# chanchanchan97/ICAFusion

Hardware: NVIDIA H100
Metric: 640x512 RGB+IR pairs/sec end-to-end (higher is better)
Workload: dtype f16

## Files before the change

### icafusion_b200/csrc/conv_common.cuh

```cuda
#pragma once
#include "icaf_internal.cuh"

namespace icaf {

constexpr int BM = 128;
constexpr int BK = 64;
constexpr int kLag = 2;
constexpr int kThreads = 288;

enum AMode { A_GATHER = 0, A_TMA2D = 1, A_TMA4D = 2 };

struct ConvProblem {
  const __half* x; const float* bias; const __half* res; __half* y;
  const float* alpha; const float* beta;
  long long x_ld, res_ld, y_ld;
  const float2* ln_stats;
  const float* ln_s;
  float2* stats_out;
};
struct ConvParams {
  ConvProblem p[2];
  int M, N, K, k_pad;
  int B, Hi, Wi, Cin, Ho, Wo, kh, kw, stride, pad;
  int act, epi;
  int a_mode, tw, th, tiles_x, tiles_y;
  int stages;
  int splits;
  int cblk;
  int ln_parts;
  float ln_eps, ln_inv_k;
  int m_tiles, n_tiles, tiles;
};
struct ConvMaps {
  CUtensorMap w[2];
  CUtensorMap a[2];
  CUtensorMap y[2];
  CUtensorMap res[2];
};

__device__ __forceinline__ ConvProblem pick_problem(const ConvParams& P, unsigned z) {
  ConvProblem r;
  r.x = z ? P.p[1].x : P.p[0].x;          r.bias = z ? P.p[1].bias : P.p[0].bias;
  r.res = z ? P.p[1].res : P.p[0].res;    r.y = z ? P.p[1].y : P.p[0].y;
  r.alpha = z ? P.p[1].alpha : P.p[0].alpha; r.beta = z ? P.p[1].beta : P.p[0].beta;
  r.x_ld = z ? P.p[1].x_ld : P.p[0].x_ld; r.res_ld = z ? P.p[1].res_ld : P.p[0].res_ld;
  r.y_ld = z ? P.p[1].y_ld : P.p[0].y_ld;
  r.ln_stats = z ? P.p[1].ln_stats : P.p[0].ln_stats; r.ln_s = z ? P.p[1].ln_s : P.p[0].ln_s;
  r.stats_out = z ? P.p[1].stats_out : P.p[0].stats_out;
  return r;
}

struct TileOrigin { int m0, tb, oy0, ox0; };
__device__ __forceinline__ void tile_origin(const ConvParams& P, int mtile, int& m0, int& tb, int& oy0, int& ox0) {
  m0 = mtile * BM; tb = 0; oy0 = 0; ox0 = 0;
  if (P.a_mode == A_TMA4D) {
    const int per_img = P.tiles_x * P.tiles_y;
    m0 = 0;
    tb = mtile / per_img;
    const int t = mtile - tb * per_img;
    oy0 = (t / P.tiles_x) * P.th;
    ox0 = (t % P.tiles_x) * P.tw;
  }
}

struct EpiRow {
  float ln_a, ln_mu;
  const float* ln_s;
  float sum, sumsq;
};
__device__ __forceinline__ void epi_row_ln(EpiRow& ex, const ConvParams& P, const ConvProblem& pr, int m, bool mvalid) {
  float su = 0.f, sq = 0.f;
  if (mvalid) {
    const float2* sp = pr.ln_stats + size_t(m) * P.ln_parts;
    for (int i = 0; i < P.ln_parts; ++i) { const float2 v = __ldg(sp + i); su += v.x; sq += v.y; }
  }
  const float mu = su * P.ln_inv_k;
  ex.ln_mu = mu;
  ex.ln_a = rsqrtf(fmaxf(sq * P.ln_inv_k - mu * mu, 0.f) + P.ln_eps);
}
__device__ __forceinline__ void epi_row_emit(const EpiRow& ex, const ConvParams& P, const ConvProblem& pr, int m, int n_begin, int n_end) {
  const int slots = (P.N + 31) >> 5;
  float2* sp = pr.stats_out + size_t(m) * slots;
  const int s0 = n_begin >> 5, s1 = min((n_end + 31) >> 5, slots);
  for (int i = s0; i < s1; ++i) sp[i] = i == s0 ? make_float2(ex.sum, ex.sumsq) : make_float2(0.f, 0.f);
// ... 77 lines not shown
__device__ __forceinline__ void epi_dispatch(int mode_act, const uint32_t (&acc)[32], const float* sb, float rbias, float alpha,
                                             float beta, const __half* rp, __half* yp, bool vec, int ncols, EpiRow& ex, int cb) {
  if (XM) {
    switch (mode_act) {
      case 9: epi_chunk<0, 0, 1>(acc, sb, rbias, alpha, beta, rp, yp, vec, ncols, ex, cb); break;
      case 10: epi_chunk<2, 0, 1>(acc, sb, rbias, alpha, beta, rp, yp, vec, ncols, ex, cb); break;
      default: epi_chunk<0, 2, 2>(acc, sb, rbias, alpha, beta, rp, yp, vec, ncols, ex, cb); break;
    }
  } else {
    switch (mode_act) {
      case 0: epi_chunk<0, 0>(acc, sb, rbias, alpha, beta, rp, yp, vec, ncols, ex, cb); break;
      case 1: epi_chunk<0, 1>(acc, sb, rbias, alpha, beta, rp, yp, vec, ncols, ex, cb); break;
      case 2: epi_chunk<0, 2>(acc, sb, rbias, alpha, beta, rp, yp, vec, ncols, ex, cb); break;
      case 3: epi_chunk<1, 0>(acc, sb, rbias, alpha, beta, rp, yp, vec, ncols, ex, cb); break;
      case 4: epi_chunk<1, 1>(acc, sb, rbias, alpha, beta, rp, yp, vec, ncols, ex, cb); break;
      case 5: epi_chunk<1, 2>(acc, sb, rbias, alpha, beta, rp, yp, vec, ncols, ex, cb); break;
      case 6: epi_chunk<2, 0>(acc, sb, rbias, alpha, beta, rp, yp, vec, ncols, ex, cb); break;
      case 7: epi_chunk<2, 1>(acc, sb, rbias, alpha, beta, rp, yp, vec, ncols, ex, cb); break;
      default: epi_chunk<2, 2>(acc, sb, rbias, alpha, beta, rp, yp, vec, ncols, ex, cb); break;
    }
  }
}

struct ConvPlan {
  int kernel;
  int bn;
  unsigned grid_x, grid_y, grid_z, cluster;
  int smem;
  int tiles, m_tiles, n_tiles;
  int sms;
  bool persist;
  int ctas;
};

}
```

### icafusion_b200/csrc/conv_gemm.cu

```cuda
#include <cstdlib>
#include <cstring>

#include "conv_common.cuh"

namespace icaf {

constexpr int kMaxStages = 10;
template <int BN>
struct SmemLayout {
  static constexpr int kABytes = BM * BK * 2;
  static constexpr int kBBytes = BN * BK * 2;
  static constexpr int kStageBytes = kABytes + kBBytes;
  static constexpr int kPitch = BN + 4;
  static constexpr int kAccBytes = BM * kPitch * 4;
  static constexpr int kTailBytes = 256 + BN * 4 + 1024;
  __host__ __device__ static int region(int stages) { return stages * kStageBytes > kAccBytes ? stages * kStageBytes : kAccBytes; }
  static int total(int stages) { return region(stages) + kTailBytes; }
};


template <int BN, bool kTmaA>
__device__ __forceinline__ void load_stage(const ConvParams& P, int a_mode, uint32_t sa, uint32_t bar, uint32_t bytes,
                                           const CUtensorMap* mw, const CUtensorMap* ma, int kb, int n0, const TileOrigin& o) {
  mbar_arrive_expect_tx(bar, bytes);
  tma_load_2d(sa + SmemLayout<BN>::kABytes, mw, bar, kb * BK, n0);
  if (a_mode == A_TMA2D) {
    tma_load_2d(sa, ma, bar, kb * BK, o.m0);
  } else if (kTmaA || a_mode == A_TMA4D) {
    const int k0 = kb * BK;
    const int tap = k0 / P.Cin;
    const int ch = k0 - tap * P.Cin;
    const int ky = tap / P.kw, kx = tap - ky * P.kw;
    tma_load_4d(sa, ma, bar, ch, o.ox0 * P.stride - P.pad + kx, o.oy0 * P.stride - P.pad + ky, o.tb);
  }
}

template <int BN, bool kQuiet, class FullBar, class HandBack>
__device__ __forceinline__ int mma_loop(float (&acc0)[BN / 2], float (&acc1)[BN / 2], uint32_t smem_base, int kStages, int nkb,
                                        int s0, uint32_t ph0, FullBar full_bar, HandBack hand_back) {
  int s = s0, s_prev = s0;
  uint32_t ph = ph0;
  for (int kb = 0; kb < nkb; ++kb) {
    if (kQuiet) mbar_wait_quiet(full_bar(s), ph); else mbar_wait(full_bar(s), ph);
    const uint32_t sa = smem_base + s * SmemLayout<BN>::kStageBytes;
    wgmma_fence();
#pragma unroll
    for (int k = 0; k < BK / 16; ++k) {
      const uint64_t bd = gmma_desc_sw128(sa + SmemLayout<BN>::kABytes + 32 * k);
      wgmma_ss<0, 0>(acc0, gmma_desc_sw128(sa + 32 * k), bd, (kb | k) != 0);
      wgmma_ss<0, 0>(acc1, gmma_desc_sw128(sa + 64 * 128 + 32 * k), bd, (kb | k) != 0);
    }
    wgmma_commit();
    wgmma_wait<1>();
    if (kb > 0) hand_back(s_prev);
    s_prev = s;
    if (++s == kStages) { s = 0; ph ^= 1; }
  }
  return s_prev;
}

template <int BN, bool XM>
__global__ void __launch_bounds__(kThreads, (BN <= 64 ? 2 : 1))
conv_gemm_tc_kernel(const ConvParams P, const __grid_constant__ ConvMaps maps) {
  extern __shared__ uint8_t smem_raw[];
  const uint32_t smem_base = (smem_u32(smem_raw) + 1023u) & ~1023u;
  using L = SmemLayout<BN>;
  const int kStages = P.stages;
  const uint32_t bar_off = uint32_t(L::region(kStages));
  const uint32_t bar_base = smem_base + bar_off;
  auto full_bar = [&](int s) { return bar_base + 8u * s; };
  auto empty_bar = [&](int s) { return bar_base + 8u * (kMaxStages + s); };
  uint8_t* smem_gen = smem_raw + (smem_base - smem_u32(smem_raw));

  pdl_launch_dependents();
  const int warp = threadIdx.x >> 5;
  const int tid = threadIdx.x;
  const int splits = P.splits;
  const int mtile = splits > 1 ? blockIdx.x / splits : blockIdx.x;
  const int ntile = blockIdx.y, bz = blockIdx.z;
  const ConvProblem pr = pick_problem(P, bz);
  const int n0 = ntile * BN;
  const int a_mode = P.a_mode;
  const uint32_t crank = splits > 1 ? cluster_ctarank() : 0u;
  const int nkb_all = P.k_pad / BK;
  const int kb_begin = (nkb_all * int(crank)) / splits;
  const int nkb = (nkb_all * (int(crank) + 1)) / splits - kb_begin;
  int m0, tb, oy0, ox0;
  tile_origin(P, mtile, m0, tb, oy0, ox0);
  const TileOrigin o{m0, tb, oy0, ox0};

  if (tid == 0) {
    const uint32_t nfull = a_mode == A_GATHER ? 129u : 1u;
    for (int s = 0; s < kStages; ++s) {
      mbar_init(full_bar(s), nfull);
      mbar_init(empty_bar(s), 4);
    }
    fence_mbar_init();
  }
  if (warp == 8 && lane_id() == 0) {
    tma_prefetch_desc(bz ? &maps.w[1] : &maps.w[0]);
    if (a_mode != A_GATHER) tma_prefetch_desc(bz ? &maps.a[1] : &maps.a[0]);
  }
  float* sbias = reinterpret_cast<float*>(smem_gen + bar_off + 256);
  float* sacc = reinterpret_cast<float*>(smem_gen);
  __syncthreads();
  pdl_wait();

  if (warp < 4) {
    float bias_r[(BN + 127) / 128];
#pragma unroll
    for (int i = 0; i < (BN + 127) / 128; ++i) {
      const int col = tid + 128 * i;
      bias_r[i] = (col < BN && pr.bias && !(P.epi & ICAF_EPI_BIAS_ROW) && n0 + col < P.N) ? __ldg(pr.bias + n0 + col) : 0.f;
    }
    float alpha = 0.f, beta = 1.f;
    if (P.epi & ICAF_EPI_SCALED_RES) { alpha = __ldg(pr.alpha); beta = __ldg(pr.beta); }
    if (a_mode == A_GATHER) {
      const int lag = kStages - 2 < kLag ? kStages - 2 : kLag;
      const int c = tid & 7;
      const int r0 = tid >> 3;
      const uint32_t sw = uint32_t(c ^ (r0 & 7)) << 4;
      uint32_t base[8];
      int iy0[8], ix0[8];
#pragma unroll
      for (int i = 0; i < 8; ++i) {
        int m = o.m0 + r0 + 16 * i;
        bool mv = m < P.M;
        int mm = mv ? m : 0;
        int ox = mm % P.Wo;
        int t = mm / P.Wo;
        int oy = t % P.Ho;
        int b = t / P.Ho;
        base[i] = uint32_t(b) * uint32_t(P.Hi * P.Wi);
        iy0[i] = mv ? oy * P.stride - P.pad : -100000;
        ix0[i] = ox * P.stride - P.pad;
      }
      int s = 0, s_done = 0;
      uint32_t ph = 0;
      for (int kb = 0; kb < nkb; ++kb) {
        mbar_wait(empty_bar(s), ph ^ 1);
        const uint32_t sa = smem_base + s * L::kStageBytes;
        const int k0 = (kb_begin + kb) * BK + c * 8;
        const bool kvalid = k0 < P.K;
        const int tap = k0 / P.Cin;
        const int ch = k0 - tap * P.Cin;
        const int ky = tap / P.kw;
        const int kx = tap - ky * P.kw;
#pragma unroll
        for (int i = 0; i < 8; ++i) {
          int iy = iy0[i] + ky, ix = ix0[i] + kx;
          bool ok = kvalid && (unsigned)iy < (unsigned)P.Hi && (unsigned)ix < (unsigned)P.Wi;
          size_t off = ok ? (size_t(base[i] + uint32_t(iy * P.Wi + ix)) * size_t(pr.x_ld) + ch) : 0;
          cp_async16(sa + uint32_t(r0 + 16 * i) * 128u + sw, pr.x + off, ok);
        }
        cp_async_commit();
        if (kb >= lag) {
          if (lag == 2) cp_async_wait<2>(); else if (lag == 1) cp_async_wait<1>(); else cp_async_wait<0>();
          fence_proxy_async_smem();
          mbar_arrive(full_bar(s_done));
          if (++s_done == kStages) s_done = 0;
        }
        if (++s == kStages) { s = 0; ph ^= 1; }
      }
      cp_async_wait<0>();
      fence_proxy_async_smem();
      for (int kb = nkb - lag < 0 ? 0 : nkb - lag; kb < nkb; ++kb) {
        mbar_arrive(full_bar(s_done));
        if (++s_done == kStages) s_done = 0;
      }
    }

    const int row = tid;
    int m;
    bool mvalid;
    if (a_mode == A_TMA4D) {
      const int ry = row / P.tw, rx = row - ry * P.tw;
      m = (tb * P.Ho + oy0 + ry) * P.Wo + ox0 + rx;
      mvalid = ry < P.th && oy0 + ry < P.Ho;
    } else {
      m = m0 + row;
      mvalid = m < P.M;
    }
    const float rbias = ((P.epi & ICAF_EPI_BIAS_ROW) && pr.bias && mvalid) ? __ldg(pr.bias + m) : 0.f;
    __half* yrow = pr.y + size_t(mvalid ? m : 0) * pr.y_ld;
    const __half* rrow = pr.res ? pr.res + size_t(mvalid ? m : 0) * pr.res_ld : nullptr;
    const int mode = (P.epi & ICAF_EPI_SCALED_RES) ? 2 : (rrow ? 1 : 0);
    if (rrow && mvalid) {
      for (int cb = 0; cb < BN && n0 + cb < P.N; cb += 64) prefetch_l2(rrow + n0 + cb);
    }
#pragma unroll
    for (int i = 0; i < (BN + 127) / 128; ++i)
      if (tid + 128 * i < BN) sbias[tid + 128 * i] = bias_r[i];
    EpiRow ex;
// ... 18 lines not shown
            float4 v;
            ld_cluster_v4(peer + 16u * q, v);
            acc[4 * q] = __float_as_uint(__uint_as_float(acc[4 * q]) + v.x);
            acc[4 * q + 1] = __float_as_uint(__uint_as_float(acc[4 * q + 1]) + v.y);
            acc[4 * q + 2] = __float_as_uint(__uint_as_float(acc[4 * q + 2]) + v.z);
            acc[4 * q + 3] = __float_as_uint(__uint_as_float(acc[4 * q + 3]) + v.w);
          }
        }
        const int nb = n0 + cb;
        if (mvalid && nb < P.N) {
          const int ncols = min(32, P.N - nb);
          const bool vec = ncols == 32 && ((reinterpret_cast<uintptr_t>(yrow + nb) & 15) == 0) &&
                           (!rrow || (reinterpret_cast<uintptr_t>(rrow + nb) & 15) == 0);
          const float* sb = sbias + cb;
          const __half* rp = rrow ? rrow + nb : nullptr;
          __half* yp = yrow + nb;
          epi_dispatch<XM>(mode_act, acc, sb, rbias, alpha, beta, rp, yp, vec, ncols, ex, cb);
        }
      }
      if (XM && mode_act == 11 && mvalid && n0 < P.N) epi_row_emit(ex, P, pr, m, n0, min(n0 + BN, P.N));
    }
    if (splits > 1) { cluster_arrive(); cluster_wait(); }
  } else if (warp < 8) {
    float acc0[BN / 2], acc1[BN / 2];
#pragma unroll
    for (int i = 0; i < BN / 2; ++i) { acc0[i] = 0.f; acc1[i] = 0.f; }
    mma_loop<BN, false>(acc0, acc1, smem_base, kStages, nkb, 0, 0u, full_bar,
                        [&](int s) { if (lane_id() == 0) mbar_arrive(empty_bar(s)); });
    wgmma_wait<0>();
    const int t = tid - 128, w = t >> 5, l = t & 31;
#pragma unroll
    for (int i = 0; i < BN / 2; i += 2) {
      const int r = 16 * w + (l >> 2) + 8 * ((i >> 1) & 1), col = 8 * (i >> 2) + 2 * (l & 3);
      *reinterpret_cast<float2*>(sacc + size_t(r) * L::kPitch + col) = make_float2(acc0[i], acc0[i + 1]);
      *reinterpret_cast<float2*>(sacc + size_t(r + 64) * L::kPitch + col) = make_float2(acc1[i], acc1[i + 1]);
    }
    if (splits > 1) { cluster_arrive(); cluster_wait(); cluster_arrive(); cluster_wait(); } else { named_bar_sync(1, 256); }
  } else {
    if (elect_one()) {
      const CUtensorMap* mw = bz ? &maps.w[1] : &maps.w[0];
      const CUtensorMap* ma = bz ? &maps.a[1] : &maps.a[0];
      const uint32_t a_bytes = a_mode == A_TMA2D ? L::kABytes : (a_mode == A_TMA4D ? uint32_t(P.tw * P.th) * 128u : 0u);
      const uint32_t bytes = L::kBBytes + a_bytes;
      int s = 0;
      uint32_t ph = 0;
      for (int kb = 0; kb < nkb; ++kb) {
        mbar_wait(empty_bar(s), ph ^ 1);
        load_stage<BN, false>(P, a_mode, smem_base + s * L::kStageBytes, full_bar(s), bytes, mw, ma, kb_begin + kb, n0, o);
        if (++s == kStages) { s = 0; ph ^= 1; }
      }
    }
    __syncwarp();
    if (splits > 1) { cluster_arrive(); cluster_wait(); cluster_arrive(); cluster_wait(); }
  }
}

constexpr int kPersistThreads = 384;
struct PersistLayout {
  static constexpr int kStageBytes = SmemLayout<128>::kStageBytes;
  static constexpr int kHalfBytes = BM * 64 * 2;
  static constexpr int kOutBytes = 2 * kHalfBytes;
  static constexpr int kPitch = 32 + 4;
  static constexpr int kChunkBytes = BM * kPitch * 4;
  static_assert(kChunkBytes <= kOutBytes, "the XM staged chunk lives in the output tile");
  __host__ __device__ static int bar_off(int stages) { return stages * kStageBytes + 2 * kOutBytes; }
  static int total(int stages) { return bar_off(stages) + 256 + 2 * 128 * 4 + 1024; }
};

struct PersistTile { int z, n0; TileOrigin o; };
__device__ __forceinline__ PersistTile persist_tile(const ConvParams& P, int t) {
  PersistTile pt;
  const int r = t / P.n_tiles;
  const int mtile = r % P.m_tiles;
  pt.n0 = (t - r * P.n_tiles) * 128;
  pt.z = r / P.m_tiles;
  tile_origin(P, mtile, pt.o.m0, pt.o.tb, pt.o.oy0, pt.o.ox0);
  return pt;
}

template <int CC>
__device__ __forceinline__ void stage_chunk(const float (&acc0)[64], const float (&acc1)[64], float* sacc, int w, int l) {
#pragma unroll
  for (int i = 16 * CC; i < 16 * CC + 16; i += 2) {
    const int r = 16 * w + (l >> 2) + 8 * ((i >> 1) & 1), col = 8 * (i >> 2) - 32 * CC + 2 * (l & 3);
    *reinterpret_cast<float2*>(sacc + r * PersistLayout::kPitch + col) = make_float2(acc0[i], acc0[i + 1]);
    *reinterpret_cast<float2*>(sacc + (r + 64) * PersistLayout::kPitch + col) = make_float2(acc1[i], acc1[i + 1]);
  }
}

template <int PP>
__device__ __forceinline__ void take_cols16(const float (&acc0)[64], const float (&acc1)[64], float (&v)[16]) {
#pragma unroll
  for (int e = 0; e < 8; ++e) { v[e] = acc0[8 * PP + e]; v[8 + e] = acc1[8 * PP + e]; }
}

template <int ACT, int RES>
__device__ __forceinline__ void epi_fragments(const float (&v)[16], uint32_t sa, const float* sb, const float (&rb)[4],
                                              float alpha, float beta) {
#pragma unroll
  for (int h = 0; h < 2; ++h) {
    uint32_t r[4];
    if (RES != 0) ldmatrix_x4(r, sa + 8192u * h);
#pragma unroll
    for (int k = 0; k < 4; ++k) {
      const float2 b = *reinterpret_cast<const float2*>(sb + 8 * (k >> 1));
      const float rbias = rb[2 * h + (k & 1)];
      float2 rf = make_float2(0.f, 0.f);
      if (RES != 0) rf = __half22float2(*reinterpret_cast<const __half2*>(&r[k]));
      r[k] = pack_half2(epi_value<ACT, RES>(v[8 * h + 2 * k], b.x, rbias, rf.x, alpha, beta),
                        epi_value<ACT, RES>(v[8 * h + 2 * k + 1], b.y, rbias, rf.y, alpha, beta));
    }
    stmatrix_x4(sa + 8192u * h, r);
  }
}

__device__ __forceinline__ void epi_fragments_dispatch(int mode_act, const float (&v)[16], uint32_t sa, const float* sb,
                                                       const float (&rb)[4], float alpha, float beta) {
  switch (mode_act) {
    case 0: epi_fragments<0, 0>(v, sa, sb, rb, alpha, beta); break;
    case 1: epi_fragments<0, 1>(v, sa, sb, rb, alpha, beta); break;
    case 2: epi_fragments<0, 2>(v, sa, sb, rb, alpha, beta); break;
    case 3: epi_fragments<1, 0>(v, sa, sb, rb, alpha, beta); break;
    case 4: epi_fragments<1, 1>(v, sa, sb, rb, alpha, beta); break;
    case 5: epi_fragments<1, 2>(v, sa, sb, rb, alpha, beta); break;
    case 6: epi_fragments<2, 0>(v, sa, sb, rb, alpha, beta); break;
    case 7: epi_fragments<2, 1>(v, sa, sb, rb, alpha, beta); break;
    default: epi_fragments<2, 2>(v, sa, sb, rb, alpha, beta); break;
  }
}

template <bool XM>
__global__ void __launch_bounds__(kPersistThreads, 1)
conv_gemm_persist_kernel(const ConvParams P, const __grid_constant__ ConvMaps maps) {
  extern __shared__ uint8_t smem_raw[];
  const uint32_t smem_base = (smem_u32(smem_raw) + 1023u) & ~1023u;
  using L = SmemLayout<128>;
  using PL = PersistLayout;
  const int kStages = P.stages;
  const uint32_t bar_off = uint32_t(PL::bar_off(kStages));
  const uint32_t bar_base = smem_base + bar_off;
  auto full_bar = [&](int s) { return bar_base + 8u * s; };
  auto empty_bar = [&](int s) { return bar_base + 8u * (kMaxStages + s); };
  auto order_bar = [&](int c) { return bar_base + 8u * (2 * kMaxStages + c); };
  auto res_bar = [&](int c) { return bar_base + 8u * (2 * kMaxStages + 2 + c); };
  uint8_t* smem_gen = smem_raw + (smem_base - smem_u32(smem_raw));

  pdl_launch_dependents();
  const int tid = threadIdx.x;
  const int wg = tid >> 7;
  const int nkb = P.k_pad / BK;
// ... 38 lines not shown
          load_stage<128, true>(P, a_mode, smem_base + s * L::kStageBytes, full_bar(s), bytes, mw, ma, kb, pt.n0, pt.o);
          if (++s == kStages) { s = 0; ph ^= 1; }
        }
      }
    }
    return;
  }

  setmaxnreg_inc<232>();
  const int c = wg - 1;
  const int t = tid & 127, w = t >> 5, l = t & 31;
  const int bar_id = 2 + c;
  const uint32_t sout = smem_base + uint32_t(kStages * L::kStageBytes + c * PL::kOutBytes);
  float* sacc = reinterpret_cast<float*>(smem_gen + kStages * L::kStageBytes + c * PL::kOutBytes);
  float* sbias = reinterpret_cast<float*>(smem_gen + bar_off + 256 + c * 128 * 4);
  const uint32_t half_bytes = a_mode == A_TMA2D ? uint32_t(PL::kHalfBytes) : uint32_t(P.tw * P.th) * 128u;
  for (int tile = blockIdx.x + c * gridDim.x; tile < P.tiles; tile += 2 * gridDim.x) {
    const int j = (tile - int(blockIdx.x)) / int(gridDim.x);
    const PersistTile pt = persist_tile(P, tile);
    const ConvProblem pr = pick_problem(P, pt.z);
    const int n0 = pt.n0;
    const TileOrigin& o = pt.o;
    const int halves = n0 + 64 < P.N ? 2 : 1;
    auto out_row = [&](int row, int& m, bool& valid) {
      if (a_mode == A_TMA4D) {
        const int ry = row / P.tw, rx = row - ry * P.tw;
        m = (o.tb * P.Ho + o.oy0 + ry) * P.Wo + o.ox0 + rx;
        valid = ry < P.th && o.oy0 + ry < P.Ho;
      } else {
        m = o.m0 + row;
        valid = m < P.M;
      }
    };
    const float bias_r = (pr.bias && !(P.epi & ICAF_EPI_BIAS_ROW) && n0 + t < P.N) ? __ldg(pr.bias + n0 + t) : 0.f;
    float alpha = 0.f, beta = 1.f;
    if (P.epi & ICAF_EPI_SCALED_RES) { alpha = __ldg(pr.alpha); beta = __ldg(pr.beta); }
    const int row = t;
    int m;
    bool mvalid;
    out_row(row, m, mvalid);
    const float rbias = ((P.epi & ICAF_EPI_BIAS_ROW) && pr.bias && mvalid) ? __ldg(pr.bias + m) : 0.f;
    __half* yrow = pr.y + size_t(mvalid ? m : 0) * pr.y_ld;
    const __half* rrow = pr.res ? pr.res + size_t(mvalid ? m : 0) * pr.res_ld : nullptr;
    const int mode = (P.epi & ICAF_EPI_SCALED_RES) ? 2 : (has_res ? 1 : 0);
    EpiRow ex;
    ex.sum = ex.sumsq = 0.f; ex.ln_a = 1.f; ex.ln_mu = 0.f; ex.ln_s = nullptr;
    float rb[4] = {0.f, 0.f, 0.f, 0.f};
    if (XM) {
      if (rrow && mvalid) {
        for (int cb = 0; cb < 128 && n0 + cb < P.N; cb += 64) prefetch_l2(rrow + n0 + cb);
      }
      ex.ln_s = pr.ln_s ? pr.ln_s + n0 : nullptr;
      if (P.ln_parts > 0) epi_row_ln(ex, P, pr, m, mvalid);
    } else {
      if ((P.epi & ICAF_EPI_BIAS_ROW) && pr.bias) {
#pragma unroll
        for (int q = 0; q < 4; ++q) {
          int mq;
          bool vq;
          out_row(16 * w + (l >> 2) + 8 * (q & 1) + 64 * (q >> 1), mq, vq);
          rb[q] = vq ? __ldg(pr.bias + mq) : 0.f;
        }
      }
      if (t == 0) {
        bulk_wait_group_read<0>();
        if (has_res) {
          const CUtensorMap* mr = pt.z ? &maps.res[1] : &maps.res[0];
          mbar_arrive_expect_tx(res_bar(c), uint32_t(halves) * half_bytes);
          for (int hh = 0; hh < halves; ++hh) {
            const uint32_t dst = sout + uint32_t(hh * PL::kHalfBytes);
            if (a_mode == A_TMA2D) tma_load_2d(dst, mr, res_bar(c), n0 + 64 * hh, o.m0);
            else tma_load_4d(dst, mr, res_bar(c), n0 + 64 * hh, o.ox0, o.oy0, o.tb);
          }
        }
      }
      sbias[t] = bias_r;
      named_bar_sync(bar_id, 128);
    }

    float acc0[64], acc1[64];
#pragma unroll
    for (int i = 0; i < 64; ++i) { acc0[i] = 0.f; acc1[i] = 0.f; }
    auto hand_back = [&](int s) { if (l == 0) mbar_arrive(empty_bar(s)); };
    const int g0 = j * nkb;
    const int s0 = g0 % kStages;
    const uint32_t ph0 = uint32_t(g0 / kStages) & 1u;
    if (j > 0) mbar_wait_quiet(order_bar(c), uint32_t((j >> 1) - (1 - c)) & 1u);
    const int s_last = mma_loop<128, true>(acc0, acc1, smem_base, kStages, nkb, s0, ph0, full_bar, hand_back);
    if (l == 0) mbar_arrive(order_bar(c ^ 1));
    wgmma_wait<0>();
    hand_back(s_last);

    if constexpr (!XM) {
      if (has_res) mbar_wait_quiet(res_bar(c), uint32_t(j >> 1) & 1u);
      const int mode_act = P.act * 3 + mode;
      const uint32_t sa = sout + uint32_t(16 * w + (l & 7) + 8 * ((l >> 3) & 1)) * 128u;
      const float* sb = sbias + 2 * (l & 3);
#pragma unroll 1
      for (int p = 0; p < 8; ++p) {
        float v[16];
        switch (p) {
          case 0: take_cols16<0>(acc0, acc1, v); break;
          case 1: take_cols16<1>(acc0, acc1, v); break;
          case 2: take_cols16<2>(acc0, acc1, v); break;
          case 3: take_cols16<3>(acc0, acc1, v); break;
          case 4: take_cols16<4>(acc0, acc1, v); break;
          case 5: take_cols16<5>(acc0, acc1, v); break;
          case 6: take_cols16<6>(acc0, acc1, v); break;
          default: take_cols16<7>(acc0, acc1, v); break;
        }
        const uint32_t a = sa + uint32_t(p >> 2) * uint32_t(PL::kHalfBytes) + (uint32_t((2 * (p & 3) + (l >> 4)) ^ (l & 7)) << 4);
        epi_fragments_dispatch(mode_act, v, a, sb + 16 * p, rb, alpha, beta);
      }
      fence_proxy_async_smem();
      named_bar_sync(bar_id, 128);
      if (t == 0) {
        const CUtensorMap* my = pt.z ? &maps.y[1] : &maps.y[0];
        for (int hh = 0; hh < halves; ++hh) {
          const uint32_t src = sout + uint32_t(hh * PL::kHalfBytes);
          if (a_mode == A_TMA2D) tma_store_2d(my, src, n0 + 64 * hh, o.m0);
          else tma_store_4d(my, src, n0 + 64 * hh, o.ox0, o.oy0, o.tb);
        }
        bulk_commit_group();
        if (tile + 2 * int(gridDim.x) >= P.tiles) bulk_wait_group<0>();
      }
      continue;
    }

    const int mode_act = P.ln_parts > 0 ? (P.act == ICAF_ACT_GELU ? 10 : 9) : 11;
    const float* arow = sacc + size_t(row) * PL::kPitch;
#pragma unroll 1
    for (int cc = 0; cc < 4; ++cc) {
      named_bar_sync(bar_id, 128);
      if (cc == 0) sbias[t] = bias_r;
      switch (cc) {
        case 0: stage_chunk<0>(acc0, acc1, sacc, w, l); break;
// ... 54 lines not shown
static int fill_geom(const icaf_conv_geom* g, int n_io, ConvParams& P) {
  if (!g || n_io < 1 || n_io > 2) return set_error(ICAF_ERR_BAD_ARG, "conv2d: need 1 or 2 problems");
  if (!(g->Cin == 4 || g->Cin % 8 == 0)) return set_error(ICAF_ERR_UNSUPPORTED, "conv2d: Cin must be 4 or a multiple of 8");
  if (g->Cin == 4 && (g->Wi % 2 || g->stride % 2 || g->pad % 2 || g->kw % 2))
    return set_error(ICAF_ERR_UNSUPPORTED, "conv2d: packed-image (Cin=4) path needs even Wi, stride, pad, kw");
  if (g->k_pad % 64 || g->k_pad < g->kh * g->kw * g->Cin) return set_error(ICAF_ERR_BAD_ARG, "conv2d: bad k_pad");
  if (g->w_rows < g->Cout) return set_error(ICAF_ERR_BAD_ARG, "conv2d: w_rows < Cout");
  long long M = (long long)g->B * g->Ho * g->Wo;
  if (M <= 0 || M > 0x7fffffffLL || (long long)g->B * g->Hi * g->Wi > 0x7fffffffLL)
    return set_error(ICAF_ERR_BAD_ARG, "conv2d: size out of range");
  if ((g->epi & (ICAF_EPI_ADD_RES | ICAF_EPI_SCALED_RES)) == (ICAF_EPI_ADD_RES | ICAF_EPI_SCALED_RES))
    return set_error(ICAF_ERR_BAD_ARG, "conv2d: ADD_RES and SCALED_RES are exclusive");
  if ((g->epi & ICAF_EPI_LN_FOLD) && ((g->epi & ~ICAF_EPI_LN_FOLD) != 0 || !(g->act == ICAF_ACT_NONE || g->act == ICAF_ACT_GELU) ||
                                      g->kh != 1 || g->kw != 1 || g->stride != 1 || g->pad != 0))
    return set_error(ICAF_ERR_UNSUPPORTED, "conv2d: LN_FOLD is a linear-layer (1x1) epilogue without residual, activation none / GELU");
  if ((g->epi & ICAF_EPI_EMIT_STATS) && ((g->epi & ~ICAF_EPI_EMIT_STATS) != ICAF_EPI_SCALED_RES || g->act != ICAF_ACT_NONE))
    return set_error(ICAF_ERR_UNSUPPORTED, "conv2d: EMIT_STATS rides on the SCALED_RES epilogue without activation");
  P.M = int(M); P.N = g->Cout; P.K = g->kh * g->kw * g->Cin; P.k_pad = g->k_pad;
  P.B = g->B; P.Hi = g->Hi; P.Wi = g->Wi; P.Cin = g->Cin; P.Ho = g->Ho; P.Wo = g->Wo;
  P.kh = g->kh; P.kw = g->kw; P.stride = g->stride; P.pad = g->pad; P.act = g->act; P.epi = g->epi;
  P.a_mode = A_GATHER; P.tw = P.th = P.tiles_x = P.tiles_y = 0; P.stages = 2; P.splits = 1; P.cblk = 64;
  P.ln_parts = 0; P.ln_eps = 0.f; P.ln_inv_k = 0.f;
  P.m_tiles = P.n_tiles = P.tiles = 0;
  memset(P.p, 0, sizeof(P.p));
  return ICAF_OK;
}

static int fill_params(const icaf_conv_geom* g, const icaf_conv_io* io, int n_io, ConvParams& P, const __half* (&w)[2]) {
  if (!io) return set_error(ICAF_ERR_BAD_ARG, "conv2d: null io");
  if (int rc = fill_geom(g, n_io, P)) return rc;
  for (int i = 0; i < 2; ++i) {
    const icaf_conv_io& s = io[i < n_io ? i : 0];
    bool need_res = g->epi & (ICAF_EPI_ADD_RES | ICAF_EPI_SCALED_RES);
    if (!s.x || !s.w || !s.y || (need_res && !s.res) || ((g->epi & ICAF_EPI_SCALED_RES) && (!s.alpha || !s.beta)))
      return set_error(ICAF_ERR_BAD_ARG, "conv2d: null pointer");
    if ((reinterpret_cast<uintptr_t>(s.x) & 15) || (reinterpret_cast<uintptr_t>(s.w) & 15) || (s.x_ld % 8 && g->Cin != 4) ||
        (g->Cin == 4 && s.x_ld != 4))
      return set_error(ICAF_ERR_BAD_ARG, "conv2d: x / w must be 16-byte aligned with x_ld a multiple of 8");
    if ((g->epi & ICAF_EPI_LN_FOLD) && (!s.ln_stats || !s.ln_colsum || s.ln_parts < 1 || s.ln_parts > 64))
      return set_error(ICAF_ERR_BAD_ARG, "conv2d: LN_FOLD needs ln_stats, ln_colsum and 1..64 partials per row");
    if ((g->epi & ICAF_EPI_EMIT_STATS) && !s.stats_out) return set_error(ICAF_ERR_BAD_ARG, "conv2d: EMIT_STATS needs stats_out");
    if (i > 0 && (g->epi & ICAF_EPI_LN_FOLD) && (s.ln_parts != io[0].ln_parts || s.ln_eps != io[0].ln_eps))
      return set_error(ICAF_ERR_BAD_ARG, "conv2d: grouped problems must share ln_parts / ln_eps");
    P.p[i] = ConvProblem{(const __half*)s.x, s.bias, need_res ? (const __half*)s.res : nullptr, (__half*)s.y, s.alpha, s.beta,
                         s.x_ld, s.res_ld, s.y_ld,
                         (g->epi & ICAF_EPI_LN_FOLD) ? (const float2*)s.ln_stats : nullptr,
// ... 78 lines not shown
  P.m_tiles = pl.m_tiles; P.n_tiles = pl.n_tiles; P.tiles = pl.tiles;
  pl.persist = true;
  pl.ctas = pl.tiles < pl.sms ? pl.tiles : pl.sms;
  pl.smem = PersistLayout::total(stages);
  return ICAF_OK;
}

template <int BN>
static int encode_maps(const ConvParams& P, const __half* const (&w)[2], const icaf_conv_geom* g, int n_io, bool out_maps,
                       ConvMaps& maps) {
  memset(&maps, 0, sizeof(maps));
  for (int i = 0; i < n_io; ++i) {
    int rc = encode_tmap_2d(&maps.w[i], w[i], (uint64_t)P.k_pad, (uint64_t)g->w_rows, (uint64_t)P.k_pad * 2, BK, BN);
    if (rc) return rc;
    const ConvProblem& pr = P.p[i];
    if (P.a_mode == A_TMA2D)
      rc = encode_tmap_2d(&maps.a[i], pr.x, (uint64_t)P.Cin, (uint64_t)P.M, (uint64_t)pr.x_ld * 2, BK, BM);
    else if (P.a_mode == A_TMA4D)
      rc = encode_tmap_nhwc(&maps.a[i], pr.x, P.Cin, P.Wi, P.Hi, P.B, pr.x_ld, BK, P.tw * P.stride, P.th * P.stride, P.stride,
                            P.stride);
    if (rc) return rc;
    if (out_maps) {
      auto out_map = [&](CUtensorMap* m, const __half* base, long long ld) {
        return P.a_mode == A_TMA2D ? encode_tmap_2d(m, base, (uint64_t)P.N, (uint64_t)P.M, (uint64_t)ld * 2, 64, BM)
                                   : encode_tmap_nhwc(m, base, P.N, P.Wo, P.Ho, P.B, ld, 64, P.tw, P.th, 1, 1);
      };
      if ((rc = out_map(&maps.y[i], pr.y, pr.y_ld))) return rc;
      if (pr.res && (rc = out_map(&maps.res[i], pr.res, pr.res_ld))) return rc;
    }
  }
  if (n_io == 1) { maps.w[1] = maps.w[0]; maps.a[1] = maps.a[0]; maps.y[1] = maps.y[0]; maps.res[1] = maps.res[0]; }
  return ICAF_OK;
}

template <int BN>
static int launch_conv(const ConvParams& P, const ConvPlan& pl, const __half* const (&w)[2], const icaf_conv_geom* g, int n_io,
                       cudaStream_t st) {
  const int xm = (P.epi & (ICAF_EPI_LN_FOLD | ICAF_EPI_EMIT_STATS)) ? 1 : 0;
  void (*kernel)(ConvParams, ConvMaps) = xm ? conv_gemm_tc_kernel<BN, true> : conv_gemm_tc_kernel<BN, false>;
  if (pl.persist) kernel = xm ? conv_gemm_persist_kernel<true> : conv_gemm_persist_kernel<false>;
  static bool configured[2][2][kMaxDevices] = {};
  if (int rc = configure_smem(kernel, 227 * 1024, configured[pl.persist][xm], "conv2d: cudaFuncSetAttribute")) return rc;
  ConvMaps maps;
  if (int rc = encode_maps<BN>(P, w, g, n_io, pl.persist && !xm, maps)) return rc;
  const dim3 grid = pl.persist ? dim3(unsigned(pl.ctas)) : dim3(pl.grid_x, pl.grid_y, pl.grid_z);
  launch_kc(kernel, grid, dim3(pl.persist ? kPersistThreads : kThreads), (size_t)pl.smem, st, pl.cluster, P, maps);
  return check_launch("conv2d_fwd");
}

static int plan_conv(const icaf_conv_geom* g, int n_io, int sms, ConvParams& P, ConvPlan& pl, bool persist_ok = true) {
  memset(&pl, 0, sizeof(pl));
  pl.sms = sms;
  if (sms < 1) return set_error(ICAF_ERR_BAD_ARG, "conv2d: SM count must be positive");
  plan_a_mode(g, P);
  const long long mt = P.a_mode == A_TMA4D ? (long long)P.B * P.tiles_x * P.tiles_y : (P.M + BM - 1) / BM;
  auto ctas = [&](int bn) { return mt * ((P.N + bn - 1) / bn) * n_io; };
  int bn = 32;
  if (P.N > 64 && ctas(128) >= sms) bn = 128;
  else if (P.N > 32 && ctas(64) >= sms) bn = 64;
  switch (bn) {
    case 128: {
      if (int rc = plan_tc<128>(P, n_io, pl)) return rc;
      return (persist_ok && P.a_mode != A_GATHER && P.splits == 1 && pl.tiles > sms) ? plan_persist(P, pl) : ICAF_OK;
    }
    case 64: return plan_tc<64>(P, n_io, pl);
    default: return plan_tc<32>(P, n_io, pl);
  }
// ... 16 lines not shown
  out->kernel = pl.kernel; out->bn = pl.bn; out->a_mode = P.a_mode;
  out->tile_w = P.tw; out->tile_h = P.th; out->tiles_x = P.tiles_x; out->tiles_y = P.tiles_y;
  out->cblk = P.cblk; out->halo = 0; out->stages = P.stages; out->splits = P.splits;
  out->grid_x = int(pl.grid_x); out->grid_y = int(pl.grid_y); out->grid_z = int(pl.grid_z); out->cluster = int(pl.cluster);
  out->smem_bytes = pl.smem; out->work_items = pl.tiles; out->ctas = pl.ctas;
  return ICAF_OK;
}

extern "C" int icaf_conv2d_fwd(const icaf_conv_geom* g, const icaf_conv_io* io, int n_io, void* stream) {
  ConvParams P;
  const __half* w[2];
  int rc = fill_params(g, io, n_io, P, w);
  if (rc) return rc;
  bool tma_out = true;
  for (int i = 0; i < n_io; ++i) {
    const ConvProblem& pr = P.p[i];
    tma_out = tma_out && (reinterpret_cast<uintptr_t>(pr.y) & 15) == 0 && pr.y_ld % 8 == 0 &&
              (!pr.res || ((reinterpret_cast<uintptr_t>(pr.res) & 15) == 0 && pr.res_ld % 8 == 0));
  }
  const bool xm = (P.epi & (ICAF_EPI_LN_FOLD | ICAF_EPI_EMIT_STATS)) != 0;
  ConvPlan pl;
  rc = plan_conv(g, n_io, sm_count_cached(), P, pl, xm || tma_out);
  if (rc) return rc;
  cudaStream_t st = (cudaStream_t)stream;
  switch (pl.bn) {
    case 128: return launch_conv<128>(P, pl, w, g, n_io, st);
    case 64: return launch_conv<64>(P, pl, w, g, n_io, st);
    case 32: return launch_conv<32>(P, pl, w, g, n_io, st);
    default: return set_error(ICAF_ERR_BAD_ARG, "conv2d: the planner produced an unknown tile width");
  }
}

extern "C" int icaf_conv2d_fwd_simt(const icaf_conv_geom* g, const icaf_conv_io* io, int n_io, void* stream) {
  SimtParams S;
  int rc = fill_params(g, io, n_io, S.P, S.w);
  if (rc) return rc;
  long long total = (long long)S.P.M * S.P.N;
  dim3 grid((unsigned)((total + 255) / 256), 1, n_io);
  launch_k(conv_gemm_simt_kernel, dim3(grid), dim3(256), 0, (cudaStream_t)stream, S);
  return check_launch("conv2d_fwd_simt");
}
```

Measured before the change: 1903.

## Move non-persistent conv epilogue to consumer warps with TMA output stores

```diff
diff --git a/icafusion_b200/csrc/conv_common.cuh b/icafusion_b200/csrc/conv_common.cuh
--- a/icafusion_b200/csrc/conv_common.cuh
+++ b/icafusion_b200/csrc/conv_common.cuh
@@ -30,6 +30,7 @@
   int ln_parts;
   float ln_eps, ln_inv_k;
   int m_tiles, n_tiles, tiles;
+  int tma_epi;
 };
 struct ConvMaps {
   CUtensorMap w[2];
@@ -60,6 +61,17 @@
     const int t = mtile - tb * per_img;
     oy0 = (t / P.tiles_x) * P.th;
     ox0 = (t % P.tiles_x) * P.tw;
+  }
+}
+
+__device__ __forceinline__ void tile_row(const ConvParams& P, const TileOrigin& o, int row, int& m, bool& valid) {
+  if (P.a_mode == A_TMA4D) {
+    const int ry = row / P.tw, rx = row - ry * P.tw;
+    m = (o.tb * P.Ho + o.oy0 + ry) * P.Wo + o.ox0 + rx;
+    valid = ry < P.th && o.oy0 + ry < P.Ho;
+  } else {
+    m = o.m0 + row;
+    valid = m < P.M;
   }
 }
 
@@ -183,6 +195,73 @@
   }
 }
 
+constexpr int kOutHalfBytes = BM * 64 * 2;
+
+template <int PP, int NA>
+__device__ __forceinline__ void take_cols16(const float (&acc0)[NA], const float (&acc1)[NA], float (&v)[16]) {
+  constexpr int Q = PP < NA / 8 ? PP : NA / 8 - 1;
+#pragma unroll
+  for (int e = 0; e < 8; ++e) { v[e] = acc0[8 * Q + e]; v[8 + e] = acc1[8 * Q + e]; }
+}
+
+template <int ACT, int RES>
+__device__ __forceinline__ void epi_fragments(const float (&v)[16], uint32_t sa, const float* sb, const float (&rb)[4],
+                                              float alpha, float beta) {
+#pragma unroll
+  for (int h = 0; h < 2; ++h) {
+    uint32_t r[4];
+    if (RES != 0) ldmatrix_x4(r, sa + 8192u * h);
+#pragma unroll
+    for (int k = 0; k < 4; ++k) {
+      const float2 b = *reinterpret_cast<const float2*>(sb + 8 * (k >> 1));
+      const float rbias = rb[2 * h + (k & 1)];
+      float2 rf = make_float2(0.f, 0.f);
+      if (RES != 0) rf = __half22float2(*reinterpret_cast<const __half2*>(&r[k]));
+      r[k] = pack_half2(epi_value<ACT, RES>(v[8 * h + 2 * k], b.x, rbias, rf.x, alpha, beta),
+                        epi_value<ACT, RES>(v[8 * h + 2 * k + 1], b.y, rbias, rf.y, alpha, beta));
+    }
+    stmatrix_x4(sa + 8192u * h, r);
+  }
+}
+
+__device__ __forceinline__ void epi_fragments_dispatch(int mode_act, const float (&v)[16], uint32_t sa, const float* sb,
+                                                       const float (&rb)[4], float alpha, float beta) {
+  switch (mode_act) {
+    case 0: epi_fragments<0, 0>(v, sa, sb, rb, alpha, beta); break;
+    case 1: epi_fragments<0, 1>(v, sa, sb, rb, alpha, beta); break;
+    case 2: epi_fragments<0, 2>(v, sa, sb, rb, alpha, beta); break;
+    case 3: epi_fragments<1, 0>(v, sa, sb, rb, alpha, beta); break;
+    case 4: epi_fragments<1, 1>(v, sa, sb, rb, alpha, beta); break;
+    case 5: epi_fragments<1, 2>(v, sa, sb, rb, alpha, beta); break;
+    case 6: epi_fragments<2, 0>(v, sa, sb, rb, alpha, beta); break;
+    case 7: epi_fragments<2, 1>(v, sa, sb, rb, alpha, beta); break;
+    default: epi_fragments<2, 2>(v, sa, sb, rb, alpha, beta); break;
+  }
+}
+
+template <int NA>
+__device__ __forceinline__ void epi_tile_fragments(int mode_act, const float (&acc0)[NA], const float (&acc1)[NA], uint32_t sout,
+                                                   const float* sbias, const float (&rb)[4], float alpha, float beta, int w, int l) {
+  const uint32_t sa = sout + uint32_t(16 * w + (l & 7) + 8 * ((l >> 3) & 1)) * 128u;
+  const float* sb = sbias + 2 * (l & 3);
+#pragma unroll 1
+  for (int p = 0; p < NA / 8; ++p) {
+    float v[16];
+    switch (p) {
+      case 0: take_cols16<0>(acc0, acc1, v); break;
+      case 1: take_cols16<1>(acc0, acc1, v); break;
+      case 2: take_cols16<2>(acc0, acc1, v); break;
+      case 3: take_cols16<3>(acc0, acc1, v); break;
+      case 4: take_cols16<4>(acc0, acc1, v); break;
+      case 5: take_cols16<5>(acc0, acc1, v); break;
+      case 6: take_cols16<6>(acc0, acc1, v); break;
+      default: take_cols16<7>(acc0, acc1, v); break;
+    }
+    const uint32_t a = sa + uint32_t(p >> 2) * uint32_t(kOutHalfBytes) + (uint32_t((2 * (p & 3) + (l >> 4)) ^ (l & 7)) << 4);
+    epi_fragments_dispatch(mode_act, v, a, sb + 16 * p, rb, alpha, beta);
+  }
+}
+
 struct ConvPlan {
   int kernel;
   int bn;
diff --git a/icafusion_b200/csrc/conv_gemm.cu b/icafusion_b200/csrc/conv_gemm.cu
--- a/icafusion_b200/csrc/conv_gemm.cu
+++ b/icafusion_b200/csrc/conv_gemm.cu
@@ -35,13 +35,13 @@
   }
 }
 
-template <int BN, bool kQuiet, class FullBar, class HandBack>
+template <int BN, class FullBar, class HandBack>
 __device__ __forceinline__ int mma_loop(float (&acc0)[BN / 2], float (&acc1)[BN / 2], uint32_t smem_base, int kStages, int nkb,
                                         int s0, uint32_t ph0, FullBar full_bar, HandBack hand_back) {
   int s = s0, s_prev = s0;
   uint32_t ph = ph0;
   for (int kb = 0; kb < nkb; ++kb) {
-    if (kQuiet) mbar_wait_quiet(full_bar(s), ph); else mbar_wait(full_bar(s), ph);
+    mbar_wait_quiet(full_bar(s), ph);
     const uint32_t sa = smem_base + s * SmemLayout<BN>::kStageBytes;
     wgmma_fence();
 #pragma unroll
@@ -58,6 +58,11 @@
   }
   return s_prev;
 }
+
+constexpr int kRegsLow = 80, kRegsHigh = 112;
+static_assert(128 * kRegsLow + 128 * kRegsHigh + 32 * 96 <= kThreads * 96, "register rebalance exceeds the launch budget");
+template <int BN, bool XM>
+__host__ __device__ constexpr bool rebalance_regs() { return BN == 32 || (BN == 64 && !XM); }
 
 template <int BN, bool XM>
 __global__ void __launch_bounds__(kThreads, (BN <= 64 ? 2 : 1))
@@ -88,6 +93,10 @@
   int m0, tb, oy0, ox0;
   tile_origin(P, mtile, m0, tb, oy0, ox0);
   const TileOrigin o{m0, tb, oy0, ox0};
+  const bool tma_epi = !XM && BN >= 64 && P.tma_epi != 0;
+  const bool has_res = (P.epi & (ICAF_EPI_ADD_RES | ICAF_EPI_SCALED_RES)) != 0;
+  const int s_out = nkb % kStages;
+  const uint32_t res_bar = bar_base + 8u * (2 * kMaxStages);
 
   if (tid == 0) {
     const uint32_t nfull = a_mode == A_GATHER ? 129u : 1u;
@@ -95,11 +104,16 @@
       mbar_init(full_bar(s), nfull);
       mbar_init(empty_bar(s), 4);
     }
+    mbar_init(res_bar, 1);
     fence_mbar_init();
   }
   if (warp == 8 && lane_id() == 0) {
     tma_prefetch_desc(bz ? &maps.w[1] : &maps.w[0]);
     if (a_mode != A_GATHER) tma_prefetch_desc(bz ? &maps.a[1] : &maps.a[0]);
+    if (tma_epi) {
+      tma_prefetch_desc(bz ? &maps.y[1] : &maps.y[0]);
+      if (has_res) tma_prefetch_desc(bz ? &maps.res[1] : &maps.res[0]);
+    }
   }
   float* sbias = reinterpret_cast<float*>(smem_gen + bar_off + 256);
   float* sacc = reinterpret_cast<float*>(smem_gen);
@@ -107,14 +121,15 @@
   pdl_wait();
 
   if (warp < 4) {
+    if constexpr (rebalance_regs<BN, XM>()) setmaxnreg_dec<kRegsLow>();
     float bias_r[(BN + 127) / 128];
 #pragma unroll
     for (int i = 0; i < (BN + 127) / 128; ++i) {
       const int col = tid + 128 * i;
-      bias_r[i] = (col < BN && pr.bias && !(P.epi & ICAF_EPI_BIAS_ROW) && n0 + col < P.N) ? __ldg(pr.bias + n0 + col) : 0.f;
+      bias_r[i] = (!tma_epi && col < BN && pr.bias && !(P.epi & ICAF_EPI_BIAS_ROW) && n0 + col < P.N) ? __ldg(pr.bias + n0 + col) : 0.f;
     }
     float alpha = 0.f, beta = 1.f;
-    if (P.epi & ICAF_EPI_SCALED_RES) { alpha = __ldg(pr.alpha); beta = __ldg(pr.beta); }
+    if (!tma_epi && (P.epi & ICAF_EPI_SCALED_RES)) { alpha = __ldg(pr.alpha); beta = __ldg(pr.beta); }
     if (a_mode == A_GATHER) {
       const int lag = kStages - 2 < kLag ? kStages - 2 : kLag;
       const int c = tid & 7;
@@ -138,7 +153,7 @@
       int s = 0, s_done = 0;
       uint32_t ph = 0;
       for (int kb = 0; kb < nkb; ++kb) {
-        mbar_wait(empty_bar(s), ph ^ 1);
+        mbar_wait_quiet(empty_bar(s), ph ^ 1);
         const uint32_t sa = smem_base + s * L::kStageBytes;
         const int k0 = (kb_begin + kb) * BK + c * 8;
         const bool kvalid = k0 < P.K;
@@ -169,6 +184,7 @@
         if (++s_done == kStages) s_done = 0;
       }
     }
+    if (tma_epi) return;
 
     const int row = tid;
     int m;
@@ -233,13 +249,52 @@
     }
     if (splits > 1) { cluster_arrive(); cluster_wait(); }
   } else if (warp < 8) {
+    if constexpr (rebalance_regs<BN, XM>()) setmaxnreg_inc<kRegsHigh>();
+    const int t = tid - 128, w = t >> 5, l = t & 31;
+    float alpha = 0.f, beta = 1.f;
+    float rb[4] = {0.f, 0.f, 0.f, 0.f};
+    if (tma_epi) {
+      if (t < BN) sbias[t] = (pr.bias && !(P.epi & ICAF_EPI_BIAS_ROW) && n0 + t < P.N) ? __ldg(pr.bias + n0 + t) : 0.f;
+      if (P.epi & ICAF_EPI_SCALED_RES) { alpha = __ldg(pr.alpha); beta = __ldg(pr.beta); }
+      if ((P.epi & ICAF_EPI_BIAS_ROW) && pr.bias) {
+#pragma unroll
+        for (int q = 0; q < 4; ++q) {
+          int mq;
+          bool vq;
+          tile_row(P, o, 16 * w + (l >> 2) + 8 * (q & 1) + 64 * (q >> 1), mq, vq);
+          rb[q] = vq ? __ldg(pr.bias + mq) : 0.f;
+        }
+      }
+      named_bar_sync(2, 128);
+    }
     float acc0[BN / 2], acc1[BN / 2];
 #pragma unroll
     for (int i = 0; i < BN / 2; ++i) { acc0[i] = 0.f; acc1[i] = 0.f; }
-    mma_loop<BN, false>(acc0, acc1, smem_base, kStages, nkb, 0, 0u, full_bar,
-                        [&](int s) { if (lane_id() == 0) mbar_arrive(empty_bar(s)); });
+    mma_loop<BN>(acc0, acc1, smem_base, kStages, nkb, 0, 0u, full_bar,
+                 [&](int s) { if (lane_id() == 0) mbar_arrive(empty_bar(s)); });
     wgmma_wait<0>();
-    const int t = tid - 128, w = t >> 5, l = t & 31;
+    if constexpr (!XM && BN >= 64) {
+      if (tma_epi) {
+        const uint32_t sout = smem_base + uint32_t(s_out) * L::kStageBytes;
+        if (has_res) mbar_wait_quiet(res_bar, 0);
+        const int mode = (P.epi & ICAF_EPI_SCALED_RES) ? 2 : (has_res ? 1 : 0);
+        epi_tile_fragments<BN / 2>(P.act * 3 + mode, acc0, acc1, sout, sbias, rb, alpha, beta, w, l);
+        fence_proxy_async_smem();
+        named_bar_sync(2, 128);
+        if (t == 0) {
+          const CUtensorMap* my = bz ? &maps.y[1] : &maps.y[0];
+          const int halves = (BN == 128 && n0 + 64 < P.N) ? 2 : 1;
+          for (int hh = 0; hh < halves; ++hh) {
+            const uint32_t src = sout + uint32_t(hh * kOutHalfBytes);
+            if (a_mode == A_TMA4D) tma_store_4d(my, src, n0 + 64 * hh, o.ox0, o.oy0, o.tb);
+            else tma_store_2d(my, src, n0 + 64 * hh, o.m0);
+          }
+          bulk_commit_group();
+          bulk_wait_group<0>();
+        }
+        return;
+      }
+    }
 #pragma unroll
     for (int i = 0; i < BN / 2; i += 2) {
       const int r = 16 * w + (l >> 2) + 8 * ((i >> 1) & 1), col = 8 * (i >> 2) + 2 * (l & 3);
@@ -256,9 +311,21 @@
       int s = 0;
       uint32_t ph = 0;
       for (int kb = 0; kb < nkb; ++kb) {
-        mbar_wait(empty_bar(s), ph ^ 1);
+        mbar_wait_quiet(empty_bar(s), ph ^ 1);
         load_stage<BN, false>(P, a_mode, smem_base + s * L::kStageBytes, full_bar(s), bytes, mw, ma, kb_begin + kb, n0, o);
         if (++s == kStages) { s = 0; ph ^= 1; }
+      }
+      if (tma_epi && has_res) {
+        mbar_wait_quiet(empty_bar(s), ph ^ 1);
+        const CUtensorMap* mr = bz ? &maps.res[1] : &maps.res[0];
+        const int halves = (BN == 128 && n0 + 64 < P.N) ? 2 : 1;
+        const uint32_t half_bytes = a_mode == A_TMA4D ? uint32_t(P.tw * P.th) * 128u : uint32_t(kOutHalfBytes);
+        mbar_arrive_expect_tx(res_bar, uint32_t(halves) * half_bytes);
+        for (int hh = 0; hh < halves; ++hh) {
+          const uint32_t dst = smem_base + uint32_t(s) * L::kStageBytes + uint32_t(hh * kOutHalfBytes);
+          if (a_mode == A_TMA4D) tma_load_4d(dst, mr, res_bar, n0 + 64 * hh, o.ox0, o.oy0, o.tb);
+          else tma_load_2d(dst, mr, res_bar, n0 + 64 * hh, o.m0);
+        }
       }
     }
     __syncwarp();
@@ -269,7 +336,7 @@
 constexpr int kPersistThreads = 384;
 struct PersistLayout {
   static constexpr int kStageBytes = SmemLayout<128>::kStageBytes;
-  static constexpr int kHalfBytes = BM * 64 * 2;
+  static constexpr int kHalfBytes = kOutHalfBytes;
   static constexpr int kOutBytes = 2 * kHalfBytes;
   static constexpr int kPitch = 32 + 4;
   static constexpr int kChunkBytes = BM * kPitch * 4;
@@ -296,47 +363,6 @@
     const int r = 16 * w + (l >> 2) + 8 * ((i >> 1) & 1), col = 8 * (i >> 2) - 32 * CC + 2 * (l & 3);
     *reinterpret_cast<float2*>(sacc + r * PersistLayout::kPitch + col) = make_float2(acc0[i], acc0[i + 1]);
     *reinterpret_cast<float2*>(sacc + (r + 64) * PersistLayout::kPitch + col) = make_float2(acc1[i], acc1[i + 1]);
-  }
-}
-
-template <int PP>
-__device__ __forceinline__ void take_cols16(const float (&acc0)[64], const float (&acc1)[64], float (&v)[16]) {
-#pragma unroll
-  for (int e = 0; e < 8; ++e) { v[e] = acc0[8 * PP + e]; v[8 + e] = acc1[8 * PP + e]; }
-}
-
-template <int ACT, int RES>
-__device__ __forceinline__ void epi_fragments(const float (&v)[16], uint32_t sa, const float* sb, const float (&rb)[4],
-                                              float alpha, float beta) {
-#pragma unroll
-  for (int h = 0; h < 2; ++h) {
-    uint32_t r[4];
-    if (RES != 0) ldmatrix_x4(r, sa + 8192u * h);
-#pragma unroll
-    for (int k = 0; k < 4; ++k) {
-      const float2 b = *reinterpret_cast<const float2*>(sb + 8 * (k >> 1));
-      const float rbias = rb[2 * h + (k & 1)];
-      float2 rf = make_float2(0.f, 0.f);
-      if (RES != 0) rf = __half22float2(*reinterpret_cast<const __half2*>(&r[k]));
-      r[k] = pack_half2(epi_value<ACT, RES>(v[8 * h + 2 * k], b.x, rbias, rf.x, alpha, beta),
-                        epi_value<ACT, RES>(v[8 * h + 2 * k + 1], b.y, rbias, rf.y, alpha, beta));
-    }
-    stmatrix_x4(sa + 8192u * h, r);
-  }
-}
-
-__device__ __forceinline__ void epi_fragments_dispatch(int mode_act, const float (&v)[16], uint32_t sa, const float* sb,
-                                                       const float (&rb)[4], float alpha, float beta) {
-  switch (mode_act) {
-    case 0: epi_fragments<0, 0>(v, sa, sb, rb, alpha, beta); break;
-    case 1: epi_fragments<0, 1>(v, sa, sb, rb, alpha, beta); break;
-    case 2: epi_fragments<0, 2>(v, sa, sb, rb, alpha, beta); break;
-    case 3: epi_fragments<1, 0>(v, sa, sb, rb, alpha, beta); break;
-    case 4: epi_fragments<1, 1>(v, sa, sb, rb, alpha, beta); break;
-    case 5: epi_fragments<1, 2>(v, sa, sb, rb, alpha, beta); break;
-    case 6: epi_fragments<2, 0>(v, sa, sb, rb, alpha, beta); break;
-    case 7: epi_fragments<2, 1>(v, sa, sb, rb, alpha, beta); break;
-    default: epi_fragments<2, 2>(v, sa, sb, rb, alpha, beta); break;
   }
 }
 
@@ -421,23 +447,13 @@
     const int n0 = pt.n0;
     const TileOrigin& o = pt.o;
     const int halves = n0 + 64 < P.N ? 2 : 1;
-    auto out_row = [&](int row, int& m, bool& valid) {
-      if (a_mode == A_TMA4D) {
-        const int ry = row / P.tw, rx = row - ry * P.tw;
-        m = (o.tb * P.Ho + o.oy0 + ry) * P.Wo + o.ox0 + rx;
-        valid = ry < P.th && o.oy0 + ry < P.Ho;
-      } else {
-        m = o.m0 + row;
-        valid = m < P.M;
-      }
-    };
     const float bias_r = (pr.bias && !(P.epi & ICAF_EPI_BIAS_ROW) && n0 + t < P.N) ? __ldg(pr.bias + n0 + t) : 0.f;
     float alpha = 0.f, beta = 1.f;
     if (P.epi & ICAF_EPI_SCALED_RES) { alpha = __ldg(pr.alpha); beta = __ldg(pr.beta); }
     const int row = t;
     int m;
     bool mvalid;
-    out_row(row, m, mvalid);
+    tile_row(P, o, row, m, mvalid);
     const float rbias = ((P.epi & ICAF_EPI_BIAS_ROW) && pr.bias && mvalid) ? __ldg(pr.bias + m) : 0.f;
     __half* yrow = pr.y + size_t(mvalid ? m : 0) * pr.y_ld;
     const __half* rrow = pr.res ? pr.res + size_t(mvalid ? m : 0) * pr.res_ld : nullptr;
@@ -457,7 +473,7 @@
         for (int q = 0; q < 4; ++q) {
           int mq;
           bool vq;
-          out_row(16 * w + (l >> 2) + 8 * (q & 1) + 64 * (q >> 1), mq, vq);
+          tile_row(P, o, 16 * w + (l >> 2) + 8 * (q & 1) + 64 * (q >> 1), mq, vq);
           rb[q] = vq ? __ldg(pr.bias + mq) : 0.f;
         }
       }
@@ -485,32 +501,14 @@
     const int s0 = g0 % kStages;
     const uint32_t ph0 = uint32_t(g0 / kStages) & 1u;
     if (j > 0) mbar_wait_quiet(order_bar(c), uint32_t((j >> 1) - (1 - c)) & 1u);
-    const int s_last = mma_loop<128, true>(acc0, acc1, smem_base, kStages, nkb, s0, ph0, full_bar, hand_back);
+    const int s_last = mma_loop<128>(acc0, acc1, smem_base, kStages, nkb, s0, ph0, full_bar, hand_back);
     if (l == 0) mbar_arrive(order_bar(c ^ 1));
     wgmma_wait<0>();
     hand_back(s_last);
 
     if constexpr (!XM) {
       if (has_res) mbar_wait_quiet(res_bar(c), uint32_t(j >> 1) & 1u);
-      const int mode_act = P.act * 3 + mode;
-      const uint32_t sa = sout + uint32_t(16 * w + (l & 7) + 8 * ((l >> 3) & 1)) * 128u;
-      const float* sb = sbias + 2 * (l & 3);
-#pragma unroll 1
-      for (int p = 0; p < 8; ++p) {
-        float v[16];
-        switch (p) {
-          case 0: take_cols16<0>(acc0, acc1, v); break;
-          case 1: take_cols16<1>(acc0, acc1, v); break;
-          case 2: take_cols16<2>(acc0, acc1, v); break;
-          case 3: take_cols16<3>(acc0, acc1, v); break;
-          case 4: take_cols16<4>(acc0, acc1, v); break;
-          case 5: take_cols16<5>(acc0, acc1, v); break;
-          case 6: take_cols16<6>(acc0, acc1, v); break;
-          default: take_cols16<7>(acc0, acc1, v); break;
-        }
-        const uint32_t a = sa + uint32_t(p >> 2) * uint32_t(PL::kHalfBytes) + (uint32_t((2 * (p & 3) + (l >> 4)) ^ (l & 7)) << 4);
-        epi_fragments_dispatch(mode_act, v, a, sb + 16 * p, rb, alpha, beta);
-      }
+      epi_tile_fragments<64>(P.act * 3 + mode, acc0, acc1, sout, sbias, rb, alpha, beta, w, l);
       fence_proxy_async_smem();
       named_bar_sync(bar_id, 128);
       if (t == 0) {
@@ -611,6 +609,7 @@
   P.a_mode = A_GATHER; P.tw = P.th = P.tiles_x = P.tiles_y = 0; P.stages = 2; P.splits = 1; P.cblk = 64;
   P.ln_parts = 0; P.ln_eps = 0.f; P.ln_inv_k = 0.f;
   P.m_tiles = P.n_tiles = P.tiles = 0;
+  P.tma_epi = 0;
   memset(P.p, 0, sizeof(P.p));
   return ICAF_OK;
 }
@@ -735,7 +734,7 @@
     if (rc) return rc;
     if (out_maps) {
       auto out_map = [&](CUtensorMap* m, const __half* base, long long ld) {
-        return P.a_mode == A_TMA2D ? encode_tmap_2d(m, base, (uint64_t)P.N, (uint64_t)P.M, (uint64_t)ld * 2, 64, BM)
+        return P.a_mode != A_TMA4D ? encode_tmap_2d(m, base, (uint64_t)P.N, (uint64_t)P.M, (uint64_t)ld * 2, 64, BM)
                                    : encode_tmap_nhwc(m, base, P.N, P.Wo, P.Ho, P.B, ld, 64, P.tw, P.th, 1, 1);
       };
       if ((rc = out_map(&maps.y[i], pr.y, pr.y_ld))) return rc;
@@ -755,7 +754,7 @@
   static bool configured[2][2][kMaxDevices] = {};
   if (int rc = configure_smem(kernel, 227 * 1024, configured[pl.persist][xm], "conv2d: cudaFuncSetAttribute")) return rc;
   ConvMaps maps;
-  if (int rc = encode_maps<BN>(P, w, g, n_io, pl.persist && !xm, maps)) return rc;
+  if (int rc = encode_maps<BN>(P, w, g, n_io, (pl.persist && !xm) || P.tma_epi, maps)) return rc;
   const dim3 grid = pl.persist ? dim3(unsigned(pl.ctas)) : dim3(pl.grid_x, pl.grid_y, pl.grid_z);
   launch_kc(kernel, grid, dim3(pl.persist ? kPersistThreads : kThreads), (size_t)pl.smem, st, pl.cluster, P, maps);
   return check_launch("conv2d_fwd");
@@ -818,6 +817,7 @@
   ConvPlan pl;
   rc = plan_conv(g, n_io, sm_count_cached(), P, pl, xm || tma_out);
   if (rc) return rc;
+  P.tma_epi = (!pl.persist && !xm && tma_out && P.splits == 1 && pl.bn >= 64) ? 1 : 0;
   cudaStream_t st = (cudaStream_t)stream;
   switch (pl.bn) {
     case 128: return launch_conv<128>(P, pl, w, g, n_io, st);
```

New measurement: 1993, median of 6. 4.7% higher.
